# janinethoma/soft_contrastive_learning

Hardware: AMD Instinct MI355X
Metric: train-step images/sec (VGG16-NetVLAD soft-MS, 640x480) (higher is better)
Workload: dtype bf16; 1 GPU; configs[1]: wms soft-contrastive train step, VGG16-NetVLAD K=64, 24 images/GPU 640x480, bf16 backbone, float32-accurate NetVLAD + f32 loss; global_batch=24, locations=1200, parallelism=dp1, optimizer=adam

## Files before the change

### soft_contrastive_learning_amd/csrc/convh.hip

```cpp
#include <mutex>

#include "conv_lds.h"
#include "conv_pack_layout.h"

namespace {

constexpr int HBW = 40;
constexpr int HWC = HBW + 2;
constexpr int HPIX = 32;
constexpr int HCCH = 32;
constexpr int HNB = 128;
constexpr int HTPB = 3;
constexpr int HWT = 4 * HNB * 8;
constexpr int HTHR = 512;
constexpr int HX = 1;

template <int BHv>
struct HCfg {
  static constexpr int BH = BHv == 24 ? 12 : BHv;
  static constexpr int WR = BH + 2;
  static constexpr int SLOTS = WR * HWC * 4;
  static constexpr int NI = (SLOTS + 511) / 512;
  static constexpr int NA = (NI + 1) / 2;
  static constexpr int WIN = NI * 8 * 512;
  static constexpr int NMT = BH / 2 * 5;
  static constexpr int MT = BHv == 24 ? 15 : BH == 12 ? 8 : BH == 8 ? 10 : 4;
  static constexpr int NT = (BHv == 24 || BH == 8) ? 2 : 4;
  static constexpr int SPT = BHv == 24 ? 3 : 2;
  static constexpr int MH = MT / SPT;
  static constexpr size_t LDS = (2 * (size_t)WIN + 3 * HTPB * (size_t)HWT) * 2;
};

template <int V>
struct HConst {
  static constexpr int value = V;
};

__device__ __forceinline__ int ht_row(int i) { return (i >= 4 && i < 12) ? 1 : 0; }
__device__ __forceinline__ int ht_col(int i) { return i < 4 ? i : i < 8 ? i - 4 : i < 12 ? i - 4 : i - 8; }

__global__ __launch_bounds__(256) void convh_pack_kernel(const void* __restrict__ w, int64_t sk,
                                                         int64_t sc, int64_t sh, int64_t sw,
                                                         int flags, int cin, int kout,
                                                         unsigned short* __restrict__ packed) {
  const int transposed = flags & 1, wf32 = flags & 2;
  const int64_t idx = (int64_t)blockIdx.x * 256 + threadIdx.x;
  const int64_t total = (int64_t)9 * (cin / HCCH) * kout * HCCH;
  if (idx >= total) return;
  const int64_t off = pack_src_offset(pack_lds_coord(idx, cin), sk, sc, sh, sw, transposed);
  packed[idx] = weight_bf16(w, off, wf32);
}

template <int EPI, int BHv, bool STAMP = false, bool FULL = false>
__global__ __launch_bounds__(HTHR, 1) void convh_kernel(const unsigned short* __restrict__ x,
                                                       const unsigned short* __restrict__ packed,
                                                       int B, int H, int W, int cin, int kout,
                                                       unsigned short* __restrict__ out,
                                                       const float* __restrict__ bias, int relu,
                                                       const unsigned short* __restrict__ mask,
                                                       unsigned char* __restrict__ pidx,
                                                       int vblocks) {
  using G = HCfg<BHv>;
  constexpr int BH = G::BH, WR = G::WR, WIN = G::WIN, NMT = G::NMT, MT = G::MT, NT = G::NT;
  constexpr int MH = G::MH, NI = G::NI, NA = G::NA, SPT = G::SPT;
  constexpr bool WEAVE = BHv == 24 || BHv == 6 || BHv == 8;
  constexpr int HS = 9 * SPT;
  extern __shared__ __attribute__((aligned(16))) unsigned short lds[];
  unsigned short* win = lds;
  unsigned short* wts = lds + 2 * WIN;
  const int lane = threadIdx.x & 63;
  const int wid = __builtin_amdgcn_readfirstlane(threadIdx.x >> 6);
  const int i = lane & 15, g = lane >> 4;
  const int kb = kout / HNB;
  const int blocks_x = (W + HBW - 1) / HBW, blocks_y = (H + BH - 1) / BH;
  const int CC = cin / HCCH, S = 9 * CC;
  const unsigned short* zeros = reinterpret_cast<const unsigned short*>(zero_block);
  int nb = 0, b = 0, y0 = 0, x0 = 0;
  int rel[NI];
#pragma unroll
  for (int n = 0; n < NI; ++n) {
    const int slot = 64 * (wid + 8 * n) + lane;
    const int pix = slot >> 2, row = pix / HWC, col = pix - row * HWC;
    const int piece = (slot & 3) ^ (((col >> 2) & 1) | ((row & 1) << 1));
    rel[n] = pix >= WR * HWC ? -1 : (row << 16) | (col << 8) | piece;
  }
  int woff[NI];
  auto locate = [&](int vb) -> bool {
    const int grp = vb / (8 * kb), rem = vb - grp * 8 * kb;
    const int pblk = grp * 8 + (rem & 7);
    nb = rem >> 3;
    if (pblk >= B * blocks_x * blocks_y) return false;
    b = pblk / (blocks_x * blocks_y);
    const int t2 = pblk % (blocks_x * blocks_y);
    y0 = (t2 / blocks_x) * BH;
    x0 = (t2 % blocks_x) * HBW;
#pragma unroll
    for (int n = 0; n < NI; ++n) {
      int r = rel[n];
      asm volatile("" : "+v"(r));
      const int y = y0 - 1 + (r >> 16), xx = x0 - 1 + ((r >> 8) & 255);
      const bool inimg = r >= 0 && y >= 0 && y < H && xx >= 0 && xx < W;
      woff[n] = inimg ? ((b * H + y) * W + xx) * cin + 8 * (r & 255) : -1;
    }
    return true;
  };
  auto issue_win = [&](int cc, int buf, int n0, int n1) {
    const unsigned base = lds_byte_of(win) + buf * WIN * 2;
#pragma unroll
    for (int n = 0; n < NI; ++n)
      if (n >= n0 && n < n1)
        glds16(woff[n] >= 0 ? x + woff[n] + HCCH * cc : zeros, base + (wid + 8 * n) * 1024);
  };
  auto issue_wts = [&](int grp, int buf) {
    const unsigned short* src = packed + ((int64_t)nb * S + HTPB * grp) * HWT + lane * 8;
    const unsigned base = lds_byte_of(wts) + buf * HTPB * HWT * 2;
#pragma unroll
    for (int n = 0; n < 3; ++n) {
      const int j = wid + 8 * n;
      glds16(src + j * 512, base + j * 1024);
    }
  };
  auto issue_wts_one = [&](int grp, int buf, int n) {
    const unsigned short* src = packed + ((int64_t)nb * S + HTPB * grp) * HWT + lane * 8;
    const unsigned base = lds_byte_of(wts) + buf * HTPB * HWT * 2;
    const int j = wid + 8 * n;
    glds16(src + j * 512, base + j * 1024);
  };
  auto stage_first = [&]() {
    issue_wts(0, 0);
    issue_wts(1, 1);
    issue_win(0, 0, 0, NI);
  };
  const int mg = NT == 4 ? wid >> 1 : wid >> 2, ng = NT == 4 ? wid & 1 : wid & 3;
  constexpr bool REG = MT % 5 == 0;
  constexpr bool ALLT = NMT % MT == 0;
  int aoff[MT];
#pragma unroll
  for (int j = 0; j < MT; ++j) {
    const int mt = MT * mg + j < NMT ? MT * mg + j : NMT - 1;
    aoff[j] = ((2 * (mt / 5)) * HWC + 8 * (mt % 5)) * HPIX;
  }
  const int lane_a = (ht_row(i) * HWC + ht_col(i)) * HPIX + (REG ? 2 * (MT / 5) * mg * HWC * HPIX : 0);
  int pieces = 0;
#pragma unroll
  for (int t = 0; t < 9; ++t) {
    const int r = ht_row(i) + t / 3, c = ht_col(i) + t % 3;
    pieces |= (g ^ (((c >> 2) & 1) | ((r & 1) << 1))) << (2 * t);
  }
  const int lane_b = (g * HNB + 16 * NT * ng + i) * 8;

  const int relu_in = relu;
  const int dbg = STAMP ? 0 : SCL_DIAG_ONLY(relu >> 1);
  relu &= 1;
  const short relu_floor = relu ? (short)0 : (short)-32768;
  bool staged = false;
  if (!STAMP && (dbg & 4) && wid >= 4) __builtin_amdgcn_s_setprio(1);
  uint64_t stamp[STAMP ? 24 : 1];
  int tcount = 0;
#define HSTAMP(k)                                                                     \
  if (STAMP)                                                                          \
  asm volatile("s_memtime %0\n\ts_waitcnt lgkmcnt(0)" : "=s"(stamp[STAMP ? (k) : 0])::"memory")
  for (int vb = blockIdx.x; vb < vblocks; vb += gridDim.x) {
    HSTAMP(0);
    if (!staged) {
      if (!locate(vb)) continue;
      stage_first();
    }
    staged = false;
    const int nb_t = nb, b_t = b, y0_t = y0, x0_t = x0;

    f32x4 acc[MT][NT];
#pragma unroll
    for (int j = 0; j < MT; ++j)
#pragma unroll
      for (int n = 0; n < NT; ++n) acc[j][n] = f32x4{0.f, 0.f, 0.f, 0.f};

    u32x4 af[2][MH], bf[2][NT];
    int tb = 0;
    auto load_half = [&](const unsigned short* wbase, int h, int par, int apar) {
      const int t = h / SPT, mh = h % SPT;
      if (mh == 0) {
        const unsigned short* wbp = wts + t * HWT + lane_b;
#pragma unroll
        for (int n = 0; n < NT; ++n)
          bf[(t + par) & 1][n] = *reinterpret_cast<const u32x4*>(wbp + 16 * n * 8);
        int pk = pieces;
        asm volatile("" : "+v"(pk));
        tb = lane_a + ((pk >> (2 * t)) & 3) * 8;
      }
#pragma unroll
      for (int j = 0; j < MH; ++j)
        af[(h + apar) & 1][j] = *reinterpret_cast<const u32x4*>(
            wbase + tb +
            (REG ? (2 * ((MH * mh + j) / 5) * HWC + 8 * ((MH * mh + j) % 5)) * HPIX : aoff[MH * mh + j]) +
            ((t / 3) * HWC + t % 3) * HPIX);
    };
    const int NG = 3 * CC;
    auto chunk = [&](int cc, auto par_c) {
      constexpr int PAR = decltype(par_c)::value;
      constexpr int APAR = PAR * (HS & 1);
      const unsigned short* wcur = win + (cc & 1) * WIN;
      const unsigned short* wnext = win + ((cc + 1) & 1) * WIN;
      const int ccn = cc + 1 < CC ? cc + 1 : cc;
      auto issue_op = [&](int gi, int k) {
        if (k < 3) {
          const int gn = 3 * cc + gi + 2 < NG ? 3 * cc + gi + 2 : NG - 3 + (gi + 2) % 3;
          issue_wts_one(gn, (gi + 2) % 3, k);
        } else {
          const int n = (gi == 0 ? 0 : NA) + k - 3;
          if (gi == 0 && n < NA) issue_win(ccn, (cc + 1) & 1, n, n + 1);
          if (gi == 1 && n < NI) issue_win(ccn, (cc + 1) & 1, n, n + 1);
        }
      };
#pragma unroll
      for (int h = 0; h < HS; ++h) {
        if (h + 1 < HS)
          load_half(wcur, h + 1, PAR, APAR);
        else
          load_half(wnext, 0, PAR ^ 1, APAR ^ (HS & 1));
        __builtin_amdgcn_sched_barrier(0);
        const int t = h / SPT, mh = h % SPT;
        const bool after_barrier = WEAVE && (h % (3 * SPT) == HX + 1);
#pragma unroll
        for (int j = 0; j < MH; ++j) {
#pragma unroll
          for (int n = 0; n < NT; ++n)
            acc[MH * mh + j][n] =
                EPI == 3 ? mfma16b(af[(h + APAR) & 1][j], bf[(t + PAR) & 1][n], acc[MH * mh + j][n])
                         : mfma16b(bf[(t + PAR) & 1][n], af[(h + APAR) & 1][j], acc[MH * mh + j][n]);
          if (after_barrier) {
            __builtin_amdgcn_sched_barrier(0);
#pragma unroll
            for (int k = j * 6 / MH; k < (j + 1) * 6 / MH; ++k) issue_op(h / (3 * SPT), k);
            __builtin_amdgcn_sched_barrier(0);
          }
        }
        if (h % (3 * SPT) == HX) {
          __builtin_amdgcn_sched_barrier(0);
          const int gi = h / (3 * SPT);
          if (gi == 1)
            asm volatile("s_waitcnt vmcnt(%0)" ::"n"(NA) : "memory");
          else
            asm volatile("s_waitcnt vmcnt(0)" ::: "memory");
          HSTAMP(2 + 9 * PAR + 3 * gi);
          __builtin_amdgcn_s_barrier();
          HSTAMP(2 + 9 * PAR + 3 * gi + 1);
          if (!WEAVE) {
            const int gn = 3 * cc + gi + 2 < NG ? 3 * cc + gi + 2 : NG - 3 + (gi + 2) % 3;
            issue_wts(gn, (gi + 2) % 3);
            if (gi == 0) issue_win(ccn, (cc + 1) & 1, 0, NA);
            if (gi == 1) issue_win(ccn, (cc + 1) & 1, NA, NI);
          }
          HSTAMP(2 + 9 * PAR + 3 * gi + 2);
        }
      }
    };

    if (!(dbg & 1)) {
      asm volatile("s_waitcnt vmcnt(0)" ::: "memory");
      __syncthreads();
    }
    HSTAMP(1);
    load_half(win, 0, 0, 0);
#pragma unroll 1
    for (int cc = 0; cc < CC; cc += 2) {
      chunk(cc, HConst<0>());
      chunk(cc + 1, HConst<1>());
    }

    int nb_e = nb_t, b_e = b_t, y0_e = y0_t, x0_e = x0_t;
    asm volatile("" : "+s"(nb_e), "+s"(b_e), "+s"(y0_e), "+s"(x0_e));
    HSTAMP(20);
    __builtin_amdgcn_s_barrier();
    HSTAMP(21);
    constexpr int SLD = 16 * NT + 8;
    constexpr int PCS = 2 * NT;
    constexpr int RR = 16 * PCS / 64;
    constexpr int SCRW = 16 * SLD + 8 * (16 * NT + 16);
    static_assert(4 * SCRW <= WIN && 4 * SCRW <= HTPB * HWT, "epilogue scratch must fit");
    unsigned short* scr = wid < 4 ? lds + WIN + wid * SCRW : wts + 2 * HTPB * HWT + (wid - 4) * SCRW;
    const int ch_w = HNB * nb_e + 16 * NT * ng;
    f32x4 bias4[EPI == 1 ? NT : 1];
    float bias1[EPI == 3 ? NT : 1];
    if (EPI == 1) {
#pragma unroll
      for (int n = 0; n < NT; ++n)
        bias4[n] = *reinterpret_cast<const f32x4*>(bias + ch_w + 16 * n + 4 * g);
    }
    if (EPI == 3) {
#pragma unroll
      for (int n = 0; n < NT; ++n) bias1[n] = bias[ch_w + 16 * n + i];
    }
    int piece_o[RR], piece_px[RR];
#pragma unroll
    for (int rr = 0; rr < RR; ++rr) {
      const int pp = lane + 64 * rr;
      piece_px[rr] = pp / PCS;
      piece_o[rr] = (ht_row(pp / PCS) * W + ht_col(pp / PCS)) * kout + 8 * (pp % PCS);
    }
    constexpr int PD = MT / 2;
    u32x4 mk[EPI == 2 ? MT : 1][EPI == 2 ? RR : 1];
    const int64_t tile_off = (((int64_t)b_e * H + y0_e) * W + x0_e) * kout + ch_w;
    const bool full_tile = FULL ? !(dbg & 2) : (y0_e + BH <= H && x0_e + HBW <= W && !(dbg & 2));
    auto load_mask = [&](int j) {
      const int mt = MT * mg + j;
      const int oy = y0_e + 2 * (mt / 5), ox = x0_e + 8 * (mt % 5);
      const unsigned short* mb = mask + tile_off + ((2 * (mt / 5)) * W + 8 * (mt % 5)) * kout;
#pragma unroll
      for (int rr = 0; rr < RR; ++rr) {
        if (FULL ? (ALLT || mt < NMT) : (full_tile && mt < NMT)) {
          mk[EPI == 2 ? j : 0][EPI == 2 ? rr : 0] = *reinterpret_cast<const u32x4*>(mb + piece_o[rr]);
        } else if (FULL) {
          mk[EPI == 2 ? j : 0][EPI == 2 ? rr : 0] = u32x4{0u, 0u, 0u, 0u};
        } else {
          const bool inside = mt < NMT && oy + ht_row(piece_px[rr]) < H && ox + ht_col(piece_px[rr]) < W;
          mk[EPI == 2 ? j : 0][EPI == 2 ? rr : 0] =
              inside ? *reinterpret_cast<const u32x4*>(mb + piece_o[rr]) : u32x4{0u, 0u, 0u, 0u};
        }
      }
    };
    if (EPI == 2) {
#pragma unroll
      for (int j = 0; j < PD; ++j) load_mask(j);
    }

    auto stage_next = [&]() {
      const int vn = vb + gridDim.x;
      if (vn < vblocks && locate(vn)) {
        asm volatile("s_waitcnt vmcnt(0)" ::: "memory");
        stage_first();
        staged = true;
      }
    };
    if (EPI != 2) stage_next();

    if (EPI == 3) {
      const int PH = H / 2, PW = W / 2;
      const bool upper = g == 0 || g == 3;
      const int cb = g < 2 ? 0 : 4;
      unsigned char* scr8 = reinterpret_cast<unsigned char*>(scr + 16 * SLD);
      constexpr int SLD8 = 16 * NT + 16;
#pragma unroll
      for (int jb = 0; jb < MT; jb += 4) {
#pragma unroll
        for (int jj = 0; jj < 4; ++jj) {
          const int j = jb + jj < MT ? jb + jj : MT - 1;
#pragma unroll
          for (int n = 0; n < NT; ++n) {
#pragma unroll
            for (int q0 = 0; q0 < 4; q0 += 2) {
              const float v0 = acc[j][n][q0], v1 = acc[j][n][q0 + 1];
              const float lm = fmaxf(v0, v1);
              const int li = v0 >= v1 ? 0 : 1;
              const float om = __shfl_xor(lm, 16);
              const int oi = __shfl_xor(li, 16);
              const float mu = upper ? lm : om, ml = upper ? om : lm;
              const int iu = upper ? li : oi, il = upper ? oi : li;
              const float m = fmaxf(mu, ml);
              const int k = mu >= ml ? iu : 2 + il;
              const int pl = 4 * jj + ((cb + q0) >> 1);
              if (upper) {
                scr[pl * SLD + 16 * n + i] = f32_to_bf16(fmaxf(m + bias1[n], 0.f));
                scr8[pl * SLD8 + 16 * n + i] = (unsigned char)k;
              }
            }
          }
        }
        __builtin_amdgcn_wave_barrier();
#pragma unroll
        for (int rr = 0; rr < RR; ++rr) {
          const int pp = lane + 64 * rr, pl = pp / PCS, pc = pp % PCS;
          const int mt = MT * mg + jb + (pl >> 2);
          const int py = (y0_e >> 1) + mt / 5, px = (x0_e >> 1) + 4 * (mt % 5) + (pl & 3);
          const u32x4 v = *reinterpret_cast<const u32x4*>(scr + pl * SLD + 8 * pc);
          if (jb + (pl >> 2) < MT && (FULL ? (ALLT || mt < NMT) : (mt < NMT && py < PH && px < PW && !(dbg & 2))))
            *reinterpret_cast<u32x4*>(out + (((int64_t)b_e * PH + py) * PW + px) * kout + ch_w + 8 * pc) = v;
        }
        if (lane < 16 * NT) {
          const int pl = lane / NT, pc = lane % NT;
          const int mt = MT * mg + jb + (pl >> 2);
          const int py = (y0_e >> 1) + mt / 5, px = (x0_e >> 1) + 4 * (mt % 5) + (pl & 3);
          const u32x4 v = *reinterpret_cast<const u32x4*>(scr8 + pl * SLD8 + 16 * pc);
          if (jb + (pl >> 2) < MT && (FULL ? (ALLT || mt < NMT) : (mt < NMT && py < PH && px < PW && !(dbg & 2))))
            *reinterpret_cast<u32x4*>(pidx + (((int64_t)b_e * PH + py) * PW + px) * kout + ch_w + 16 * pc) = v;
        }
        __builtin_amdgcn_wave_barrier();
      }
    } else {
      unsigned short* out_tile = out + tile_off;
#pragma unroll
      for (int j = 0; j < MT; ++j) {
        const int mt = MT * mg + j;
        if (ALLT || mt < NMT) {
          const int oy = y0_e + 2 * (mt / 5), ox = x0_e + 8 * (mt % 5);
          unsigned short* ob = out_tile + ((2 * (mt / 5)) * W + 8 * (mt % 5)) * kout;
#pragma unroll
          for (int n = 0; n < NT; ++n) {
            f32x4 v = acc[j][n];
            if (EPI == 1) v += bias4[n];
            unsigned p0 = pack2_bf16(v[0], v[1]), p1 = pack2_bf16(v[2], v[3]);
            if (EPI == 1) {
              p0 = max2_i16(p0, relu_floor);
              p1 = max2_i16(p1, relu_floor);
            }
            const u32x2 pk = {p0, p1};
            *reinterpret_cast<u32x2*>(scr + i * SLD + 16 * n + 4 * g) = pk;
          }
          __builtin_amdgcn_wave_barrier();
#pragma unroll
          for (int rr = 0; rr < RR; ++rr) {
            u32x4 v = *reinterpret_cast<const u32x4*>(scr + piece_px[rr] * SLD + 8 * ((lane + 64 * rr) % PCS));
            if (EPI == 2) v = relu_mask(v, mk[EPI == 2 ? j : 0][EPI == 2 ? rr : 0]);
            if (full_tile) {
              *reinterpret_cast<u32x4*>(ob + piece_o[rr]) = v;
            } else if (!FULL) {
              const bool inside = oy + ht_row(piece_px[rr]) < H && ox + ht_col(piece_px[rr]) < W && !(dbg & 2);
              if (inside) *reinterpret_cast<u32x4*>(ob + piece_o[rr]) = v;
            }
          }
          __builtin_amdgcn_wave_barrier();
        }
        if (EPI == 2) {
          __builtin_amdgcn_sched_barrier(0);
          if (j + PD < MT) load_mask(j + PD);
          if (j + PD == MT - 1) stage_next();
          __builtin_amdgcn_sched_barrier(0);
        }
      }
    }
    if (STAMP) {
      HSTAMP(22);
      if (threadIdx.x == 64 * ((relu_in >> 4) & 7) && (tcount == 1 || tcount == 2)) {
        uint64_t* o = reinterpret_cast<uint64_t*>(out + (int64_t)B * H * W * kout) +
                      (int64_t)(blockIdx.x * 2 + tcount - 1) * 24;
#pragma unroll
        for (int k = 0; k < 23; ++k) o[k] = stamp[STAMP ? k : 0];
      }
      ++tcount;
    }
  }
#undef HSTAMP
}

}

struct HGeom {
  const unsigned short* packed;
  int bh;
  LdsConvGrid grid;
};

template <int E, int BHV, bool STAMP = false, bool FULL = false>
static void convh_run(const LdsConvCall& c, const HGeom& g, int relu) {
  if constexpr (!STAMP && !FULL)
    if (c.H % HCfg<BHV>::BH == 0 && c.W % HBW == 0) return convh_run<E, BHV, false, true>(c, g, relu);
  static SclDeviceOnce once;
  scl_call_once(once, [] {
    (void)hipFuncSetAttribute(reinterpret_cast<const void*>(&convh_kernel<E, BHV, STAMP, FULL>),
                              hipFuncAttributeMaxDynamicSharedMemorySize, (int)HCfg<BHV>::LDS);
  });
  SCL_LAUNCH("convh_kernel", (convh_kernel<E, BHV, STAMP, FULL>), dim3(g.grid.gsize), dim3(HTHR),
             HCfg<BHV>::LDS, c.stream, (const unsigned short*)c.x, g.packed, c.B, c.H, c.W, c.cin,
             c.kout, (unsigned short*)c.out, c.bias, relu, (const unsigned short*)c.mask,
             (unsigned char*)c.pidx, g.grid.vblocks);
}
template <int BHV>
static void convh_epilogue(const LdsConvCall& c, const HGeom& g, int dbgbits) {
  if (c.pidx) convh_run<3, BHV>(c, g, dbgbits);
  else if (c.mask) convh_run<2, BHV>(c, g, dbgbits);
  else if (c.bias) convh_run<1, BHV>(c, g, (c.relu ? 1 : 0) | dbgbits);
  else convh_run<0, BHV>(c, g, 0);
}

#ifdef SCL_DIAG
static bool convh_diag(const LdsConvCall& c, const HGeom& g, int* rc);
#endif

int convh_launch(const LdsConvCall& c) {
  const int dv = SCL_DIAG_ONLY(c.dv);
  HGeom g;
  g.packed = (const unsigned short*)c.workspace;
  if (c.flags & SCL_W_PACKED) {
    g.packed = (const unsigned short*)c.w;
  } else {
    const int64_t total = (int64_t)9 * (c.cin / HCCH) * c.kout * HCCH;
    SCL_LAUNCH("convh_pack_kernel", convh_pack_kernel, dim3((unsigned)((total + 255) / 256)),
               dim3(256), 0, c.stream, c.w, c.sk, c.sc, c.sh, c.sw, c.flags, c.cin, c.kout,
               (unsigned short*)c.workspace);
  }
  const int bx = (c.W + HBW - 1) / HBW, kb = c.kout / HNB;
  const int cus = scl_conv_cus();
  g.bh = 12;
  int64_t best = -1;
  for (int cand : {12, 8, 6}) {
    const int64_t wg = (int64_t)c.B * ((c.H + cand - 1) / cand) * bx * kb;
    const int64_t cost = ((wg + cus - 1) / cus) * (cand + 2);
    if (best < 0 || cost < best) {
      best = cost;
      g.bh = cand;
    }
  }
  if (dv == 3012 || dv == 3008 || dv == 3006) g.bh = dv - 3000;
  if (dv == 3013) g.bh = 12;
  g.grid = lds_conv_grid((int64_t)c.B * ((c.H + g.bh - 1) / g.bh) * bx, kb, cus, dv);
#ifdef SCL_DIAG
  {
    int rc;
    if (convh_diag(c, g, &rc)) return rc;
  }
#endif
  const int dbgbits = (dv >= 3020 && dv < 3024) ? (dv - 3020) << 1 : (dv == 3040 ? 4 << 1 : 0);
  if (g.bh == 12) convh_epilogue<24>(c, g, dbgbits);
  else if (g.bh == 8) convh_epilogue<8>(c, g, dbgbits);
  else convh_epilogue<6>(c, g, dbgbits);
  return scl_launch_status();
}
```

### soft_contrastive_learning_amd/csrc/convh_diag.hip

```cpp
#include "convh.hip"

static bool convh_diag(const LdsConvCall& c, const HGeom& g, int* rc) {
  const int dv = c.dv;
  const bool stamps = dv >= 3024 && dv < 3040 && c.bias && !c.mask && !c.pidx && g.bh == 12;
  if (dv != 3012 && !stamps) return false;
  if (dv == 3012)
    convh_epilogue<12>(c, g, 0);
  else if (dv < 3032)
    convh_run<1, 24, true>(c, g, (c.relu ? 1 : 0) | ((dv - 3024) << 4));
  else
    convh_run<1, 12, true>(c, g, (c.relu ? 1 : 0) | ((dv - 3032) << 4));
  *rc = scl_launch_status();
  return true;
}
```

Before: 2080 images/sec.

## Add paired 6-row tile mode to convh sharing weight loads across two spatial blocks

Adds a PAIR configuration (BHv=66) where one workgroup stages two 6-row spatial blocks in its LDS window. Each half of the waves computes one block, so each weight tile loaded into LDS is reused for twice the output pixels. The BH heuristic now costs this candidate alongside 12/8/6 and picks it when its cost is lower. It adds a dump slot for surplus DMA pieces and a liveness guard on stores for an odd trailing block. It also adds a NODMA diagnostic variant.

After: 2027 images/sec. 0.975x the previous value.

```diff
diff --git a/soft_contrastive_learning_amd/csrc/convh.hip b/soft_contrastive_learning_amd/csrc/convh.hip
--- a/soft_contrastive_learning_amd/csrc/convh.hip
+++ b/soft_contrastive_learning_amd/csrc/convh.hip
@@ -15,26 +15,37 @@
 constexpr int HTHR = 512;
 constexpr int HX = 1;
 
+constexpr size_t HLDS_MAX = 160 * 1024;
+
 template <int BHv>
 struct HCfg {
-  static constexpr int BH = BHv == 24 ? 12 : BHv;
+  static constexpr bool PAIR = BHv == 66;
+  static constexpr int BH = BHv == 24 ? 12 : PAIR ? 6 : BHv;
   static constexpr int WR = BH + 2;
-  static constexpr int SLOTS = WR * HWC * 4;
+  static constexpr int WRS = PAIR ? 2 * WR : WR;
+  static constexpr int SLOTS = WRS * HWC * 4;
   static constexpr int NI = (SLOTS + 511) / 512;
   static constexpr int NA = (NI + 1) / 2;
-  static constexpr int WIN = NI * 8 * 512;
+  static constexpr int NPC = PAIR ? SLOTS / 64 : NI * 8;
+  static_assert(!PAIR || SLOTS % 64 == 0, "a pair's windows must be whole DMA pieces");
+  static constexpr int WIN = NPC * 512;
+  static constexpr int DUMP = PAIR ? 512 : 0;
   static constexpr int NMT = BH / 2 * 5;
-  static constexpr int MT = BHv == 24 ? 15 : BH == 12 ? 8 : BH == 8 ? 10 : 4;
-  static constexpr int NT = (BHv == 24 || BH == 8) ? 2 : 4;
-  static constexpr int SPT = BHv == 24 ? 3 : 2;
+  static constexpr int MT = (BHv == 24 || PAIR) ? 15 : BH == 12 ? 8 : BH == 8 ? 10 : 4;
+  static constexpr int NT = (BHv == 24 || PAIR || BH == 8) ? 2 : 4;
+  static constexpr int SPT = (BHv == 24 || PAIR) ? 3 : 2;
   static constexpr int MH = MT / SPT;
-  static constexpr size_t LDS = (2 * (size_t)WIN + 3 * HTPB * (size_t)HWT) * 2;
+  static constexpr size_t LDS = (2 * (size_t)WIN + 3 * HTPB * (size_t)HWT + DUMP) * 2;
+  static_assert(LDS <= HLDS_MAX, "window buffers + weight buffers (+ dump) must fit a CU's LDS");
 };
+static_assert(HCfg<66>::LDS == 2 * 43008 + 3 * 24576 + 1024, "pair: 42 + 42 window pieces, 72 weight pieces, 1 dump");
 
 template <int V>
 struct HConst {
   static constexpr int value = V;
 };
+
+__device__ __forceinline__ int hsel(bool c, int a, int b) { return __builtin_amdgcn_readfirstlane(c ? a : b); }
 
 __device__ __forceinline__ int ht_row(int i) { return (i >= 4 && i < 12) ? 1 : 0; }
 __device__ __forceinline__ int ht_col(int i) { return i < 4 ? i : i < 8 ? i - 4 : i < 12 ? i - 4 : i - 8; }
@@ -51,7 +62,7 @@
   packed[idx] = weight_bf16(w, off, wf32);
 }
 
-template <int EPI, int BHv, bool STAMP = false, bool FULL = false>
+template <int EPI, int BHv, bool STAMP = false, bool FULL = false, bool NODMA = false>
 __global__ __launch_bounds__(HTHR, 1) void convh_kernel(const unsigned short* __restrict__ x,
                                                        const unsigned short* __restrict__ packed,
                                                        int B, int H, int W, int cin, int kout,
@@ -63,7 +74,8 @@
   using G = HCfg<BHv>;
   constexpr int BH = G::BH, WR = G::WR, WIN = G::WIN, NMT = G::NMT, MT = G::MT, NT = G::NT;
   constexpr int MH = G::MH, NI = G::NI, NA = G::NA, SPT = G::SPT;
-  constexpr bool WEAVE = BHv == 24 || BHv == 6 || BHv == 8;
+  constexpr bool PAIR = G::PAIR;
+  constexpr bool WEAVE = BHv == 24 || BHv == 6 || BHv == 8 || PAIR;
   constexpr int HS = 9 * SPT;
   extern __shared__ __attribute__((aligned(16))) unsigned short lds[];
   unsigned short* win = lds;
@@ -76,40 +88,58 @@
   const int CC = cin / HCCH, S = 9 * CC;
   const unsigned short* zeros = reinterpret_cast<const unsigned short*>(zero_block);
   int nb = 0, b = 0, y0 = 0, x0 = 0;
+  int bB = 0, y0B = 0, x0B = 0;
+  int liveB = 0;
   int rel[NI];
 #pragma unroll
   for (int n = 0; n < NI; ++n) {
     const int slot = 64 * (wid + 8 * n) + lane;
     const int pix = slot >> 2, row = pix / HWC, col = pix - row * HWC;
     const int piece = (slot & 3) ^ (((col >> 2) & 1) | ((row & 1) << 1));
-    rel[n] = pix >= WR * HWC ? -1 : (row << 16) | (col << 8) | piece;
+    rel[n] = pix >= G::WRS * HWC ? -1 : (row << 16) | (col << 8) | piece;
   }
   int woff[NI];
   auto locate = [&](int vb) -> bool {
     const int grp = vb / (8 * kb), rem = vb - grp * 8 * kb;
     const int pblk = grp * 8 + (rem & 7);
     nb = rem >> 3;
-    if (pblk >= B * blocks_x * blocks_y) return false;
-    b = pblk / (blocks_x * blocks_y);
-    const int t2 = pblk % (blocks_x * blocks_y);
+    const int per = blocks_x * blocks_y, nblk = B * per;
+    const int p0 = PAIR ? 2 * pblk : pblk;
+    if (p0 >= nblk) return false;
+    b = p0 / per;
+    const int t2 = p0 % per;
     y0 = (t2 / blocks_x) * BH;
     x0 = (t2 % blocks_x) * HBW;
+    if (PAIR) {
+      const int p1 = p0 + 1, t3 = p1 % per;
+      liveB = p1 < nblk ? 1 : 0;
+      bB = p1 / per;
+      y0B = (t3 / blocks_x) * BH;
+      x0B = (t3 % blocks_x) * HBW;
+    }
 #pragma unroll
     for (int n = 0; n < NI; ++n) {
       int r = rel[n];
       asm volatile("" : "+v"(r));
-      const int y = y0 - 1 + (r >> 16), xx = x0 - 1 + ((r >> 8) & 255);
-      const bool inimg = r >= 0 && y >= 0 && y < H && xx >= 0 && xx < W;
-      woff[n] = inimg ? ((b * H + y) * W + xx) * cin + 8 * (r & 255) : -1;
+      const int row = r >> 16;
+      const bool sB = PAIR && row >= WR;
+      const int y = (sB ? y0B - WR : y0) - 1 + row, xx = (sB ? x0B : x0) - 1 + ((r >> 8) & 255);
+      const bool inimg = r >= 0 && (!sB || liveB != 0) && y >= 0 && y < H && xx >= 0 && xx < W;
+      woff[n] = inimg ? (((sB ? bB : b) * H + y) * W + xx) * cin + 8 * (r & 255) : -1;
     }
     return true;
   };
   auto issue_win = [&](int cc, int buf, int n0, int n1) {
     const unsigned base = lds_byte_of(win) + buf * WIN * 2;
+    const unsigned dump = lds_byte_of(wts) + 3 * HTPB * HWT * 2;
 #pragma unroll
     for (int n = 0; n < NI; ++n)
-      if (n >= n0 && n < n1)
-        glds16(woff[n] >= 0 ? x + woff[n] + HCCH * cc : zeros, base + (wid + 8 * n) * 1024);
+      if (n >= n0 && n < n1) {
+        unsigned dst = base + (wid + 8 * n) * 1024;
+        if (PAIR && 8 * n + 7 >= G::NPC)
+          dst = __builtin_amdgcn_readfirstlane(wid + 8 * n >= G::NPC ? dump : dst);
+        glds16(woff[n] >= 0 ? x + woff[n] + HCCH * cc : zeros, dst);
+      }
   };
   auto issue_wts = [&](int grp, int buf) {
     const unsigned short* src = packed + ((int64_t)nb * S + HTPB * grp) * HWT + lane * 8;
@@ -140,7 +170,8 @@
     const int mt = MT * mg + j < NMT ? MT * mg + j : NMT - 1;
     aoff[j] = ((2 * (mt / 5)) * HWC + 8 * (mt % 5)) * HPIX;
   }
-  const int lane_a = (ht_row(i) * HWC + ht_col(i)) * HPIX + (REG ? 2 * (MT / 5) * mg * HWC * HPIX : 0);
+  const int lane_a = (ht_row(i) * HWC + ht_col(i)) * HPIX + (REG ? (PAIR ? WR : 2 * (MT / 5)) * mg * HWC * HPIX : 0);
+  const int mt0 = PAIR ? 0 : MT * mg;
   int pieces = 0;
 #pragma unroll
   for (int t = 0; t < 9; ++t) {
@@ -167,7 +198,9 @@
       stage_first();
     }
     staged = false;
-    const int nb_t = nb, b_t = b, y0_t = y0, x0_t = x0;
+    const bool sB_t = PAIR && mg;
+    const int nb_t = nb, b_t = PAIR ? hsel(sB_t, bB, b) : b, y0_t = PAIR ? hsel(sB_t, y0B, y0) : y0;
+    const int x0_t = PAIR ? hsel(sB_t, x0B, x0) : x0, live_t = PAIR ? hsel(sB_t, liveB, 1) : 1;
 
     f32x4 acc[MT][NT];
 #pragma unroll
@@ -203,6 +236,7 @@
       const unsigned short* wnext = win + ((cc + 1) & 1) * WIN;
       const int ccn = cc + 1 < CC ? cc + 1 : cc;
       auto issue_op = [&](int gi, int k) {
+        if (NODMA) return;
         if (k < 3) {
           const int gn = 3 * cc + gi + 2 < NG ? 3 * cc + gi + 2 : NG - 3 + (gi + 2) % 3;
           issue_wts_one(gn, (gi + 2) % 3, k);
@@ -245,7 +279,7 @@
           HSTAMP(2 + 9 * PAR + 3 * gi);
           __builtin_amdgcn_s_barrier();
           HSTAMP(2 + 9 * PAR + 3 * gi + 1);
-          if (!WEAVE) {
+          if (!WEAVE && !NODMA) {
             const int gn = 3 * cc + gi + 2 < NG ? 3 * cc + gi + 2 : NG - 3 + (gi + 2) % 3;
             issue_wts(gn, (gi + 2) % 3);
             if (gi == 0) issue_win(ccn, (cc + 1) & 1, 0, NA);
@@ -268,8 +302,9 @@
       chunk(cc + 1, HConst<1>());
     }
 
-    int nb_e = nb_t, b_e = b_t, y0_e = y0_t, x0_e = x0_t;
-    asm volatile("" : "+s"(nb_e), "+s"(b_e), "+s"(y0_e), "+s"(x0_e));
+    int nb_e = nb_t, b_e = b_t, y0_e = y0_t, x0_e = x0_t, live_e = live_t;
+    asm volatile("" : "+s"(nb_e), "+s"(b_e), "+s"(y0_e), "+s"(x0_e), "+s"(live_e));
+    const bool live = !PAIR || live_e != 0;
     HSTAMP(20);
     __builtin_amdgcn_s_barrier();
     HSTAMP(21);
@@ -303,17 +338,17 @@
     const int64_t tile_off = (((int64_t)b_e * H + y0_e) * W + x0_e) * kout + ch_w;
     const bool full_tile = FULL ? !(dbg & 2) : (y0_e + BH <= H && x0_e + HBW <= W && !(dbg & 2));
     auto load_mask = [&](int j) {
-      const int mt = MT * mg + j;
+      const int mt = mt0 + j;
       const int oy = y0_e + 2 * (mt / 5), ox = x0_e + 8 * (mt % 5);
       const unsigned short* mb = mask + tile_off + ((2 * (mt / 5)) * W + 8 * (mt % 5)) * kout;
 #pragma unroll
       for (int rr = 0; rr < RR; ++rr) {
-        if (FULL ? (ALLT || mt < NMT) : (full_tile && mt < NMT)) {
+        if (live && (FULL ? (ALLT || mt < NMT) : (full_tile && mt < NMT))) {
           mk[EPI == 2 ? j : 0][EPI == 2 ? rr : 0] = *reinterpret_cast<const u32x4*>(mb + piece_o[rr]);
         } else if (FULL) {
           mk[EPI == 2 ? j : 0][EPI == 2 ? rr : 0] = u32x4{0u, 0u, 0u, 0u};
         } else {
-          const bool inside = mt < NMT && oy + ht_row(piece_px[rr]) < H && ox + ht_col(piece_px[rr]) < W;
+          const bool inside = live && mt < NMT && oy + ht_row(piece_px[rr]) < H && ox + ht_col(piece_px[rr]) < W;
           mk[EPI == 2 ? j : 0][EPI == 2 ? rr : 0] =
               inside ? *reinterpret_cast<const u32x4*>(mb + piece_o[rr]) : u32x4{0u, 0u, 0u, 0u};
         }
@@ -370,18 +405,18 @@
 #pragma unroll
         for (int rr = 0; rr < RR; ++rr) {
           const int pp = lane + 64 * rr, pl = pp / PCS, pc = pp % PCS;
-          const int mt = MT * mg + jb + (pl >> 2);
+          const int mt = mt0 + jb + (pl >> 2);
           const int py = (y0_e >> 1) + mt / 5, px = (x0_e >> 1) + 4 * (mt % 5) + (pl & 3);
           const u32x4 v = *reinterpret_cast<const u32x4*>(scr + pl * SLD + 8 * pc);
-          if (jb + (pl >> 2) < MT && (FULL ? (ALLT || mt < NMT) : (mt < NMT && py < PH && px < PW && !(dbg & 2))))
+          if (live && jb + (pl >> 2) < MT && (FULL ? (ALLT || mt < NMT) : (mt < NMT && py < PH && px < PW && !(dbg & 2))))
             *reinterpret_cast<u32x4*>(out + (((int64_t)b_e * PH + py) * PW + px) * kout + ch_w + 8 * pc) = v;
         }
         if (lane < 16 * NT) {
           const int pl = lane / NT, pc = lane % NT;
-          const int mt = MT * mg + jb + (pl >> 2);
+          const int mt = mt0 + jb + (pl >> 2);
           const int py = (y0_e >> 1) + mt / 5, px = (x0_e >> 1) + 4 * (mt % 5) + (pl & 3);
           const u32x4 v = *reinterpret_cast<const u32x4*>(scr8 + pl * SLD8 + 16 * pc);
-          if (jb + (pl >> 2) < MT && (FULL ? (ALLT || mt < NMT) : (mt < NMT && py < PH && px < PW && !(dbg & 2))))
+          if (live && jb + (pl >> 2) < MT && (FULL ? (ALLT || mt < NMT) : (mt < NMT && py < PH && px < PW && !(dbg & 2))))
             *reinterpret_cast<u32x4*>(pidx + (((int64_t)b_e * PH + py) * PW + px) * kout + ch_w + 16 * pc) = v;
         }
         __builtin_amdgcn_wave_barrier();
@@ -390,8 +425,8 @@
       unsigned short* out_tile = out + tile_off;
 #pragma unroll
       for (int j = 0; j < MT; ++j) {
-        const int mt = MT * mg + j;
-        if (ALLT || mt < NMT) {
+        const int mt = mt0 + j;
+        if (live && (ALLT || mt < NMT)) {
           const int oy = y0_e + 2 * (mt / 5), ox = x0_e + 8 * (mt % 5);
           unsigned short* ob = out_tile + ((2 * (mt / 5)) * W + 8 * (mt % 5)) * kout;
 #pragma unroll
@@ -447,19 +482,20 @@
 struct HGeom {
   const unsigned short* packed;
   int bh;
+  bool pair;
   LdsConvGrid grid;
 };
 
-template <int E, int BHV, bool STAMP = false, bool FULL = false>
+template <int E, int BHV, bool STAMP = false, bool FULL = false, bool NODMA = false>
 static void convh_run(const LdsConvCall& c, const HGeom& g, int relu) {
   if constexpr (!STAMP && !FULL)
     if (c.H % HCfg<BHV>::BH == 0 && c.W % HBW == 0) return convh_run<E, BHV, false, true>(c, g, relu);
   static SclDeviceOnce once;
   scl_call_once(once, [] {
-    (void)hipFuncSetAttribute(reinterpret_cast<const void*>(&convh_kernel<E, BHV, STAMP, FULL>),
+    (void)hipFuncSetAttribute(reinterpret_cast<const void*>(&convh_kernel<E, BHV, STAMP, FULL, NODMA>),
                               hipFuncAttributeMaxDynamicSharedMemorySize, (int)HCfg<BHV>::LDS);
   });
-  SCL_LAUNCH("convh_kernel", (convh_kernel<E, BHV, STAMP, FULL>), dim3(g.grid.gsize), dim3(HTHR),
+  SCL_LAUNCH("convh_kernel", (convh_kernel<E, BHV, STAMP, FULL, NODMA>), dim3(g.grid.gsize), dim3(HTHR),
              HCfg<BHV>::LDS, c.stream, (const unsigned short*)c.x, g.packed, c.B, c.H, c.W, c.cin,
              c.kout, (unsigned short*)c.out, c.bias, relu, (const unsigned short*)c.mask,
              (unsigned char*)c.pidx, g.grid.vblocks);
@@ -491,18 +527,25 @@
   const int bx = (c.W + HBW - 1) / HBW, kb = c.kout / HNB;
   const int cus = scl_conv_cus();
   g.bh = 12;
+  bool pairs = false;
   int64_t best = -1;
-  for (int cand : {12, 8, 6}) {
-    const int64_t wg = (int64_t)c.B * ((c.H + cand - 1) / cand) * bx * kb;
-    const int64_t cost = ((wg + cus - 1) / cus) * (cand + 2);
+  for (int cand : {12, 8, 66, 6}) {
+    const int bh = cand == 66 ? 6 : cand;
+    const int64_t blocks = (int64_t)c.B * ((c.H + bh - 1) / bh) * bx;
+    const int64_t wg = (cand == 66 ? (blocks + 1) / 2 : blocks) * kb;
+    const int64_t cost = ((wg + cus - 1) / cus) * (cand == 66 ? 2 * (bh + 2) : bh + 2);
     if (best < 0 || cost < best) {
       best = cost;
-      g.bh = cand;
+      g.bh = bh;
+      pairs = cand == 66;
     }
   }
   if (dv == 3012 || dv == 3008 || dv == 3006) g.bh = dv - 3000;
   if (dv == 3013) g.bh = 12;
-  g.grid = lds_conv_grid((int64_t)c.B * ((c.H + g.bh - 1) / g.bh) * bx, kb, cus, dv);
+  if (dv == 3014 || dv == 3042) g.bh = 6;
+  const int64_t pblocks = (int64_t)c.B * ((c.H + g.bh - 1) / g.bh) * bx;
+  g.pair = g.bh == 6 && (dv == 3014 || (pairs && dv != 3006 && dv != 3042));
+  g.grid = lds_conv_grid(g.pair ? (pblocks + 1) / 2 : pblocks, kb, cus, dv);
 #ifdef SCL_DIAG
   {
     int rc;
@@ -512,6 +555,7 @@
   const int dbgbits = (dv >= 3020 && dv < 3024) ? (dv - 3020) << 1 : (dv == 3040 ? 4 << 1 : 0);
   if (g.bh == 12) convh_epilogue<24>(c, g, dbgbits);
   else if (g.bh == 8) convh_epilogue<8>(c, g, dbgbits);
+  else if (g.pair) convh_epilogue<66>(c, g, dbgbits);
   else convh_epilogue<6>(c, g, dbgbits);
   return scl_launch_status();
 }
diff --git a/soft_contrastive_learning_amd/csrc/convh_diag.hip b/soft_contrastive_learning_amd/csrc/convh_diag.hip
--- a/soft_contrastive_learning_amd/csrc/convh_diag.hip
+++ b/soft_contrastive_learning_amd/csrc/convh_diag.hip
@@ -2,14 +2,29 @@
 
 static bool convh_diag(const LdsConvCall& c, const HGeom& g, int* rc) {
   const int dv = c.dv;
-  const bool stamps = dv >= 3024 && dv < 3040 && c.bias && !c.mask && !c.pidx && g.bh == 12;
-  if (dv != 3012 && !stamps) return false;
+  const bool fwd = c.bias && !c.mask && !c.pidx;
+  const bool stamps = dv >= 3024 && dv < 3040 && fwd && g.bh == 12;
+  const bool nodma = (dv == 3041 || dv == 3042) && fwd && c.H % g.bh == 0 && c.W % HBW == 0 && g.bh != 8;
+  if (dv == 3042 && !nodma) {
+    *rc = SCL_E_KIND;
+    return true;
+  }
+  if (dv != 3012 && dv != 3006 && !stamps && !nodma) return false;
+  const int relu = c.relu ? 1 : 0;
   if (dv == 3012)
     convh_epilogue<12>(c, g, 0);
+  else if (dv == 3006)
+    convh_epilogue<6>(c, g, 0);
+  else if (nodma && g.bh == 12)
+    convh_run<1, 24, false, true, true>(c, g, relu);
+  else if (nodma && g.pair)
+    convh_run<1, 66, false, true, true>(c, g, relu);
+  else if (nodma)
+    convh_run<1, 6, false, true, true>(c, g, relu);
   else if (dv < 3032)
-    convh_run<1, 24, true>(c, g, (c.relu ? 1 : 0) | ((dv - 3024) << 4));
+    convh_run<1, 24, true>(c, g, relu | ((dv - 3024) << 4));
   else
-    convh_run<1, 12, true>(c, g, (c.relu ? 1 : 0) | ((dv - 3032) << 4));
+    convh_run<1, 12, true>(c, g, relu | ((dv - 3032) << 4));
   *rc = scl_launch_status();
   return true;
 }
```
